# NoahVl/Explaining-In-Style-Reproducibility-Study

Hardware: AMD Instinct MI355X
Metric: StylEx G+D+enc train-step images/sec @256px (higher is better)
Workload: dtype bf16; 1 GPU; FFHQ-shaped 256x256 StylEx, batch 32/GPU, GAE=2 (noise+encoder micro-steps), GP every 4th step, ResNet-18 classifier; image_size=256, batch_per_gpu=32, start_step=0, gradient_accumulate_every=2, global_batch=32, parallelism=dp1

## Files before the change

explaining-in-style-reproducibility-study_amd/csrc/fused_bwd.hip:

```cpp
#include <hip/hip_runtime.h>
#include <stdint.h>
#include <stdlib.h>

#include "stylex_internal.h"

namespace {

constexpr int NT = 256;

template <int K>
struct Acc {
    float4 v[K];
    __device__ __forceinline__ void zero() {
#pragma unroll
        for (int k = 0; k < K; ++k) v[k] = make_float4(0.f, 0.f, 0.f, 0.f);
    }
};

template <int K>
__device__ __forceinline__ void block_reduce_store(Acc<K>& a, float* smem, int cv, int prow, int CV, int rpp, int C,
                                                   float* partial_row , bool active) {
    float4* s4 = reinterpret_cast<float4*>(smem);
    if (active) {
#pragma unroll
// ... 326 lines not shown
            const long o1 = two ? o + step : o;
            L8 t0 = ld8(t, o), t1 = ld8(t, o1);
            const L8 x0 = ld8(x, o), x1 = ld8(x, o1);
#pragma unroll
            for (int e = 0; e < 8; ++e) a[0].e[e] += x0.e[e] * t0.e[e];
            if (two) {
#pragma unroll
                for (int e = 0; e < 8; ++e) a[0].e[e] += x1.e[e] * t1.e[e];
            }
            if (gx) {
#pragma unroll
                for (int e = 0; e < 8; ++e) {
                    t0.e[e] *= s8.e[e];
                    t1.e[e] *= s8.e[e];
                }
                st8(gx, o, t0);
                if (two) st8(gx, o1, t1);
            }
        }
    }
    block_reduce_store8<1>(a, smem, g, C, partial + ((long)g.b * nchunks + blockIdx.x) * C);
}

inline size_t reduce_smem8(int C, int K) { return (size_t)K * (NT / (C >> 2)) * (C >> 3) * 32; }

inline bool al16(const void* p) { return (reinterpret_cast<uintptr_t>(p) & 15) == 0; }
inline bool glue_wide(int act_dtype, int C) {
    const char* env = getenv("STYLEX_GLUE_WIDE");
    return act_dtype == 1 && C % 8 == 0 && !(env && env[0] == '0');
}

inline size_t reduce_smem(int C, int K) {
    int CV = (C + 3) / 4;
    if (CV > NT) CV = NT;
    int rpp = NT / CV;
    return (size_t)K * rpp * CV * 16;
}

inline bool ok_shape(const int64_t* sh, int nchunks) {
    return sh[0] > 0 && sh[1] > 0 && sh[2] > 0 && sh[3] > 0 && sh[3] <= 1024 && (sh[3] % 4 == 0) && nchunks > 0 &&
           sh[0] <= 65535;
}

}

extern "C" {
// ... 60 lines not shown
        return (int)hipGetLastError();
    }
    hipLaunchKernelGGL(modconv_bwd_prep_kernel, dim3(nchunks, (unsigned)sh[0]), dim3(NT), reduce_smem(C, 3),
                       (hipStream_t)stream, gy, y, noise, (int)noise_stride, noise_w, noise_b, gz, partial, (int)sh[1],
                       (int)sh[2], C, nchunks, lrelu, act_dtype, gz_scale, natural);
    return (int)hipGetLastError();
}

int stylex_scale_reduce(const void* x, const void* t, const float* s, void* gx, float* partial, const int64_t* sh,
                        int nchunks, int act_dtype, void* stream) {
    if (act_dtype != 0 && act_dtype != 1) return STYLEX_EINVAL;
    if (!x || !t || !s || !partial || !ok_shape(sh, nchunks)) return STYLEX_EINVAL;
    int HW = (int)(sh[1] * sh[2]), C = (int)sh[3];
    if (glue_wide(act_dtype, C) && al16(x) && al16(t) && al16(s) && al16(gx) && al16(partial)) {
        hipLaunchKernelGGL(scale_reduce_wide_kernel, dim3(nchunks, (unsigned)sh[0]), dim3(NT8), reduce_smem8(C, 1),
                           (hipStream_t)stream, x, t, s, gx, partial, HW, C, nchunks);
        return (int)hipGetLastError();
    }
    hipLaunchKernelGGL(scale_reduce_kernel, dim3(nchunks, (unsigned)sh[0]), dim3(NT), reduce_smem(C, 1),
                       (hipStream_t)stream, x, t, s, gx, partial, HW, C, nchunks, act_dtype);
    return (int)hipGetLastError();
}

}
```

explaining-in-style-reproducibility-study_amd/stylex/hip_backend.py:

```python
import os as _os

if _os.environ.get("STYLEX_MIOPEN_ALLOW_BWD_GTC", "0") != "1":
    _os.environ.setdefault("MIOPEN_DEBUG_CONV_IMPLICIT_GEMM_ASM_BWD_GTC_XDLOPS_NHWC", "0")

import atexit
import ctypes
import os
import weakref

import torch

import operand_cache
from operand_cache import mark_updated, packs, stamp as _gen, vectors

_HERE = os.path.dirname(os.path.abspath(__file__))
LIB_PATH = os.path.join(os.path.dirname(_HERE), "libstylex_hip.so")

F32, BF16, BF16_ACT = 0, 1, 2
EPI_BIAS, EPI_LRELU, EPI_OSCALE, EPI_NOISE, EPI_RESIDUAL, EPI_RELU, EPI_GATE, EPI_NOISE_NAT = 1, 2, 4, 8, 16, 32, 64, 128
EPI_MASK_OUT, EPI_GATE_MASK = 256, 512

_c_f = ctypes.c_void_p
_i64p = ctypes.POINTER(ctypes.c_int64)

# ... 47 lines not shown
    "stylex_conv2d_bwd_weight_s2d": (ctypes.c_int, [ctypes.c_void_p, ctypes.c_void_p, _c_f, ctypes.c_void_p, ctypes.c_int64, _i64p,
                                                    ctypes.c_int, ctypes.c_float, ctypes.c_int, ctypes.c_int, ctypes.c_void_p]),
    "stylex_upsample2x_bilinear_fwd": (ctypes.c_int, [_c_f, _c_f, _i64p, ctypes.c_int, ctypes.c_void_p]),
    "stylex_upsample2x_bilinear_bwd": (ctypes.c_int, [_c_f, _c_f, _i64p, ctypes.c_int, ctypes.c_void_p]),
    "stylex_rgb_up_blur_add_fwd": (ctypes.c_int, [_c_f, _c_f, _c_f, _i64p, ctypes.c_int, ctypes.c_void_p]),
    "stylex_rgb_up_blur_add_bwd": (ctypes.c_int, [_c_f, _c_f, _i64p, ctypes.c_int, ctypes.c_void_p]),
    "stylex_blur3x3_reflect_fwd": (ctypes.c_int, [_c_f, _c_f, _i64p, ctypes.c_int, ctypes.c_void_p]),
    "stylex_blur3x3_reflect_bwd": (ctypes.c_int, [_c_f, _c_f, _i64p, ctypes.c_int, ctypes.c_void_p]),
    "stylex_bias_act_fwd": (ctypes.c_int, [_c_f, _c_f, _c_f, ctypes.c_int64, _c_f, _c_f, _c_f, _i64p, ctypes.c_int,
                                           ctypes.c_void_p]),
    "stylex_bias_act_bwd": (ctypes.c_int, [_c_f, _c_f, _c_f, _i64p, ctypes.c_int, ctypes.c_void_p]),
    "stylex_rowwise_sumsq": (ctypes.c_int, [_c_f, _c_f, _i64p, ctypes.c_void_p]),
    "stylex_reduce_chunks": (ctypes.c_int, [_i64p]),
    "stylex_act_bwd_reduce": (ctypes.c_int, [_c_f, _c_f, _c_f, _c_f, _i64p, ctypes.c_int, ctypes.c_int, ctypes.c_float,
                                             ctypes.c_int, ctypes.c_void_p]),
    "stylex_modconv_bwd_prep": (ctypes.c_int, [_c_f, _c_f, _c_f, ctypes.c_int64, _c_f, _c_f, _c_f, _c_f, _i64p,
                                               ctypes.c_int, ctypes.c_int, ctypes.c_int, ctypes.c_void_p]),
    "stylex_modconv_bwd_prep_scaled": (ctypes.c_int, [_c_f, _c_f, _c_f, ctypes.c_int64, _c_f, _c_f, _c_f, _c_f, _c_f, _i64p,
                                                      ctypes.c_int, ctypes.c_int, ctypes.c_int, ctypes.c_void_p]),
    "stylex_modconv_bwd_prep_nat": (ctypes.c_int, [_c_f, _c_f, _c_f, ctypes.c_int64, _c_f, _c_f, _c_f, _c_f, _c_f, _i64p,
                                                   ctypes.c_int, ctypes.c_int, ctypes.c_int, ctypes.c_void_p]),
    "stylex_scale_reduce": (ctypes.c_int, [_c_f, _c_f, _c_f, _c_f, _c_f, _i64p, ctypes.c_int, ctypes.c_int,
                                           ctypes.c_void_p]),
    "stylex_pad_rgb8": (ctypes.c_int, [_c_f, _c_f, _i64p, _i64p, ctypes.c_int, ctypes.c_void_p]),
    "stylex_affine_act_nchw_fwd": (ctypes.c_int, [_c_f, _c_f, _c_f, _c_f, _c_f, ctypes.c_int64, ctypes.c_int64, ctypes.c_int64,
                                                  ctypes.c_int, ctypes.c_void_p]),
    "stylex_affine_act_nchw_bwd": (ctypes.c_int, [_c_f, _c_f, _c_f, _c_f, _c_f, ctypes.c_int64, ctypes.c_int64, ctypes.c_int64,
                                                  ctypes.c_int, ctypes.c_void_p]),
    "stylex_affine_relu_maxpool_fwd": (ctypes.c_int, [_c_f, _c_f, _c_f, _c_f, _c_f, ctypes.c_int64, ctypes.c_int64,
                                                      ctypes.c_int64, ctypes.c_int64, ctypes.c_void_p]),
    "stylex_affine_relu_maxpool_bwd": (ctypes.c_int, [_c_f, _c_f, _c_f, _c_f, ctypes.c_int64, ctypes.c_int64, ctypes.c_int64,
                                                      ctypes.c_int64, ctypes.c_void_p]),
    "stylex_lpips_tap_nhwc_fwd": (ctypes.c_int, [_c_f, _c_f, _c_f, _c_f, _c_f, _c_f, ctypes.c_int64, ctypes.c_int64, ctypes.c_int64,
                                                 ctypes.c_int64, ctypes.c_void_p]),
    "stylex_lpips_tap_nhwc_bwd": (ctypes.c_int, [_c_f, _c_f, _c_f, _c_f, _c_f, _c_f, _c_f, _c_f, ctypes.c_int64, ctypes.c_int64,
                                                 ctypes.c_int64, ctypes.c_void_p]),
    "stylex_nchw_f32_to_nhwc_bf16": (ctypes.c_int, [_c_f, _c_f, ctypes.c_int64, ctypes.c_int64, ctypes.c_int64, ctypes.c_int,
                                                    ctypes.c_void_p]),
    "stylex_nhwc_bf16_to_nchw_f32": (ctypes.c_int, [_c_f, _c_f, _c_f, ctypes.c_int64, ctypes.c_int64, ctypes.c_int64, ctypes.c_void_p]),
    "stylex_resize_norm_fwd": (ctypes.c_int, [_c_f, _c_f, _c_f, _c_f, _i64p, _i64p, ctypes.c_void_p]),
    "stylex_resize_norm_bwd": (ctypes.c_int, [_c_f, _c_f, _c_f, _i64p, ctypes.c_void_p]),
    "stylex_fid_prep": (ctypes.c_int, [_c_f, _c_f, _i64p, _i64p, ctypes.c_int, ctypes.c_void_p]),
    "stylex_affine_act_nchw_slice_fwd": (ctypes.c_int, [_c_f, _c_f, _c_f, _c_f, _c_f, ctypes.c_int64, ctypes.c_int64,
                                                        ctypes.c_int64, ctypes.c_int64, ctypes.c_int, ctypes.c_void_p]),
    "stylex_fid_moments_acc": (ctypes.c_int, [_c_f, _c_f, _c_f, _c_f, ctypes.c_int64, ctypes.c_int64, ctypes.c_int64,
                                              ctypes.c_void_p]),
# ... 70 lines not shown
    "stylex_initial_block_bwd_data": (ctypes.c_int, [_c_f, _c_f, _c_f, _i64p, ctypes.c_int, ctypes.c_int, ctypes.c_void_p]),
    "stylex_initial_block_bwd_weight": (ctypes.c_int, [_c_f, _c_f, _c_f, _i64p, ctypes.c_int, ctypes.c_void_p]),
    "stylex_resample_rows_u8": (ctypes.c_int, [ctypes.c_void_p, _c_f, ctypes.c_int64, ctypes.c_int64, ctypes.c_int64, _c_f,
                                               ctypes.c_int64, _c_f, ctypes.c_int64, ctypes.c_void_p]),
    "stylex_resample_cols_u8": (ctypes.c_int, [ctypes.c_void_p, _c_f, ctypes.c_int64, ctypes.c_int64, ctypes.c_int64, _c_f,
                                               ctypes.c_int64, _c_f, ctypes.c_int64, _c_f, _c_f, ctypes.c_int64,
                                               ctypes.c_void_p]),
    "stylex_crop_lut_u8": (ctypes.c_int, [ctypes.c_void_p, _c_f, ctypes.c_int64, ctypes.c_int64, ctypes.c_int64, _c_f,
                                          ctypes.c_int64, _c_f, _c_f, ctypes.c_int64, ctypes.c_void_p]),
    "stylex_style_edit_max_k": (ctypes.c_int64, []),
    "stylex_style_edit_levels": (ctypes.c_int, [_c_f] * 9 + [ctypes.c_int64] * 5 + [ctypes.c_float, ctypes.c_void_p]),
    "stylex_timing_report": (ctypes.c_int, [ctypes.c_int, _i64p, ctypes.POINTER(ctypes.c_double),
                                            ctypes.POINTER(ctypes.c_double), ctypes.POINTER(ctypes.c_double)]),
}

_lib = None
_inited_devices = set()


class StylexHipError(RuntimeError):
    pass


OPTIONAL_SYMBOLS = frozenset(["stylex_modconv_bwd_prep_nat"])
_MISSING_OPTIONAL = set()


def has_symbol(name):
    load_library()
    return name not in _MISSING_OPTIONAL


def load_library(path=None):
    global _lib
    if _lib is not None:
        return _lib
    path = path or os.environ.get("STYLEX_HIP_LIB", LIB_PATH)
    if not os.path.isfile(path):
        raise StylexHipError("libstylex_hip.so not found at %s — run `python __graft_entry__.py build` "
                             "(there is no CPU fallback for the product path)" % path)
    lib = ctypes.CDLL(path)
    _MISSING_OPTIONAL.clear()
    for name, (res, args) in SIGNATURES.items():
        if name in OPTIONAL_SYMBOLS and path != LIB_PATH and not hasattr(lib, name):
            _MISSING_OPTIONAL.add(name)
            continue
        fn = getattr(lib, name)
# ... 1401 lines not shown
                                           _ptr(partial), shp, nch, lr, _adt(gy), _stream()), "stylex_modconv_bwd_prep")
    else:
        gz_scale = _f32(gz_scale)
        _check(lib.stylex_modconv_bwd_prep_scaled(_ptr(gy), _ptr(y), _ptr(noise), ns, _ptr(noise_w), _ptr(noise_b),
                                                  _ptr(gz_scale), _ptr(gz), _ptr(partial), shp, nch, lr, _adt(gy), _stream()),
               "stylex_modconv_bwd_prep_scaled")
    return gz, partial.sum(dim=1)


def scale_reduce(x, t, s, want_gx=True):
    lib = _ensure_device(x)
    assert is_cl(x) and is_cl(t) and x.dtype == t.dtype
    b, c, h, w = x.shape
    shp = _shape(b, h, w, c)
    nch = lib.stylex_reduce_chunks(shp)
    partial = _empty((b, nch, c), dtype=torch.float32, device=x.device)
    gx = empty_cl(tuple(x.shape), x) if want_gx else None
    s = _f32(s)
    _check(lib.stylex_scale_reduce(_ptr(x), _ptr(t), _ptr(s), _ptr(gx), _ptr(partial), shp, nch, _adt(x), _stream()),
           "stylex_scale_reduce")
    return gx, partial.sum(dim=1)


def torgb_ok(x):
    c = x.shape[1]
    if os.environ.get("STYLEX_TORGB", "1") == "0":
        return False
    return x.is_cuda and x.dtype == torch.bfloat16 and 8 <= c <= 512 and (c & (c - 1)) == 0


def torgb_fwd(x, s1, w):
    lib = _ensure_device(x)
    assert is_cl(x) and x.dtype == torch.bfloat16
    b, c, h, wd = x.shape
    y = empty_cl((b, 4, h, wd), x)
    s1, w = _f32(s1), _f32(w)
    _check(lib.stylex_torgb_fwd(_ptr(x), _ptr(s1), _ptr(w), _ptr(y), _shape(b, h, wd, c), _stream()), "stylex_torgb_fwd")
    return y


def torgb_bwd(x, gy, s1, w, want_gx=True):
    lib = _ensure_device(x)
    assert is_cl(x) and is_cl(gy) and gy.shape[1] == 4 and x.dtype == gy.dtype == torch.bfloat16
    b, c, h, wd = x.shape
    shp = _shape(b, h, wd, c)
    nch = lib.stylex_torgb_chunks(shp)
# ... 316 lines not shown
```

explaining-in-style-reproducibility-study_amd/stylex/networks.py:

```python
import atexit
import math
from math import log2

import os

import torch
import torch.nn.functional as F
from torch import nn

import ops


def exists(v):
    return v is not None


_SIDE = {}
atexit.register(_SIDE.clear)


def _side_stream(t, which=0):
    import os

    if not t.is_cuda or os.environ.get("STYLEX_STREAMS", "1") == "0":
# ... 222 lines not shown

    def forward_main(self, x, istyle, inoise, styles=None):
        if exists(self.upsample):
            x = self.upsample(x)
        coords = None
        self._rgb_style = None
        if styles is None:
            fused = ops.style_affines(istyle, self.to_style1, self.to_style2, self.to_rgb.to_style)
            if fused is not None:
                style1, style2, self._rgb_style, coords = fused
            else:
                style1, style2 = self.to_style1(istyle), self.to_style2(istyle)
        else:
            style1, style2 = styles
        x = ops.modconv_noise_act(x, style1, self.conv1.weight, inoise, self.to_noise1.weight[:, 0],
                                  self.to_noise1.bias, demod=self.conv1.demod, eps=self.conv1.eps)
        x = ops.modconv_noise_act(x, style2, self.conv2.weight, inoise, self.to_noise2.weight[:, 0],
                                  self.to_noise2.bias, demod=self.conv2.demod, eps=self.conv2.eps)
        return x, (coords if coords is not None else torch.cat([style1, style2], dim=-1))

    def forward(self, x, prev_rgb, istyle, inoise):
        x, coords = self.forward_main(x, istyle, inoise)
        rgb = self.to_rgb(x, prev_rgb, istyle, style=self.__dict__.pop("_rgb_style", None))
        return x, rgb, coords


class DiscriminatorBlock(nn.Module):
    def __init__(self, input_channels, filters, downsample=True):
        super().__init__()
        self.conv_res = HipConv2d(input_channels, filters, 1, stride=(2 if downsample else 1))
        self.net = nn.Sequential(HipConv2d(input_channels, filters, 3, padding=1, act=True), _FusedAct(),
                                 HipConv2d(filters, filters, 3, padding=1, act=True), _FusedAct())
        self.downsample = nn.Sequential(Blur(), HipConv2d(filters, filters, 3, padding=1, stride=2)) if downsample else None

    def forward(self, x):
        fused = getattr(ops.impl(), "dblock", None)
        if fused is not None:
            out = fused(x, self.conv_res, self.net[0], self.net[2], self.downsample[1] if exists(self.downsample) else None)
            if out is not None:
                return out
        side = _side_stream(x)
        if side is None:
            res = self.conv_res(x)
            x = self.net(x)
        else:
            main = torch.cuda.current_stream()
# ... 35 lines not shown
            self.initial_block = nn.Parameter(torch.randn((1, filters[0], 4, 4)))
        self.initial_conv = HipConv2d(filters[0], filters[0], 3, padding=1)
        self.blocks = nn.ModuleList([])
        self.attns = nn.ModuleList([])
        for ind in range(self.num_layers):
            self.attns.append(attn_and_ff(filters[ind]) if self.num_layers - ind in attn_layers else None)
            self.blocks.append(GeneratorBlock(latent_dim, filters[ind], filters[ind + 1], upsample=ind != 0,
                                              upsample_rgb=ind != self.num_layers - 1, rgba=transparent))

    def first_activation(self, styles):
        if self.no_const:
            return ops.initial_block(styles, self.to_initial_block.weight)
        return self.initial_block.expand(styles.shape[0], -1, -1, -1)

    def forward(self, styles, input_noise, get_style_coords=False, block_inputs=None):
        x = self.initial_conv(self.first_activation(styles))
        rgb, coords = None, []
        per_layer = styles.unbind(1)
        for li, block in enumerate(self.blocks):
            if exists(self.attns[li]):
                x = self.attns[li](x)
            if block_inputs is not None:
                block_inputs.append((x, rgb))
            x, sc = block.forward_main(x, per_layer[li], input_noise)
            coords.append(sc)
            rgb = block.to_rgb(x, rgb, per_layer[li], style=block.__dict__.pop("_rgb_style", None), padded=True)
        if rgb.shape[1] == 4 and self.blocks[0].to_rgb.conv.filters == 3:
            rgb = rgb[:, :3]
        rgb = rgb.float()
        if get_style_coords:
            return rgb, torch.cat(coords, dim=1)
        return rgb


class DiscriminatorE(nn.Module):
    def __init__(self, image_size, network_capacity=16, fq_layers=[], fq_dict_size=256, attn_layers=[],
                 transparent=False, encoder=False, encoder_dim=512, fmap_max=512, conditional=False):
        super().__init__()
        assert not fq_layers, "the fq variant is out of scope (SURVEY §2a)"
        filters = discriminator_filters(image_size, network_capacity, fmap_max, transparent)
        n = len(filters) - 1
        blocks, attn_blocks = [], []
        for i in range(n):
            blocks.append(DiscriminatorBlock(filters[i], filters[i + 1], downsample=i != n - 1))
            attn_blocks.append(attn_and_ff(filters[i + 1]) if i + 1 in attn_layers else None)
        self.blocks = nn.ModuleList(blocks)
        self.attn_blocks = nn.ModuleList(attn_blocks)
        self.quantize_blocks = nn.ModuleList([None] * n)
        chan_last = filters[-1]
# ... 20 lines not shown
```

explaining-in-style-reproducibility-study_amd/stylex/ops.py:

```python
import collections
import math

import os

import torch
from contextlib import nullcontext as _nullcontext
import torch.nn.functional as F

import hip_backend as hb

_PRECISION = hb.F32


_NAMES = {"fp32": hb.F32, "f32": hb.F32, "bf16": hb.BF16_ACT, "bf16_f32act": hb.BF16}


def set_precision(name):
    global _PRECISION
    _PRECISION = _NAMES[name]


def get_precision():
    return {hb.F32: "fp32", hb.BF16_ACT: "bf16", hb.BF16: "bf16_f32act"}[_PRECISION]

# ... 478 lines not shown


def _natural_noise(inoise):
    hit = _NAT_NOISE.get("k")
    if (hit is not None and hit[0] is inoise and hit[1] == inoise._version
            and not (inoise.is_cuda and torch.cuda.is_current_stream_capturing())):
        return hit[2]
    nat = inoise[:, :, :, 0].transpose(1, 2).contiguous().float()
    _NAT_NOISE["k"] = (inoise, inoise._version, nat)
    return nat


class _ModConvFast(torch.autograd.Function):

    @staticmethod
    def forward(ctx, x, s1, d, w, noise, nw, nb, pad, lrelu, noise_nat=None):
        x = _cl(x)
        pre = _PRECISION == hb.BF16_ACT and s1 is not None and x.shape[2] * x.shape[3] <= 64 and x.shape[1] % 64 == 0
        ctx.pre = pre
        if pre:
            x_in, s_in = (x.float() * s1[:, :, None, None]).to(x.dtype).contiguous(memory_format=torch.channels_last), None
        else:
            x_in, s_in = x, s1
        if noise_nat is not None and noise_nat.shape[1] % 4 == 0:
            y = hb.conv2d_fwd(x_in, w, 1, pad, _PRECISION, in_scale=s_in, out_scale=d, noise=noise_nat, noise_w=nw,
                              noise_b=nb, lrelu=lrelu, noise_natural=True)
        else:
            y = hb.conv2d_fwd(x_in, w, 1, pad, _PRECISION, in_scale=s_in, out_scale=d, noise=noise, noise_w=nw, noise_b=nb,
                              lrelu=lrelu)
        ctx.save_for_backward(x, s1, d, w, noise, nw, nb, y if (lrelu or d is not None or noise is not None) else None,
                              noise_nat)
        ctx.cfg = (pad, lrelu)
        return y

    @staticmethod
    @torch.autograd.function.once_differentiable
    def backward(ctx, gy):
        x, s1, d, w, noise, nw, nb, y, noise_nat = ctx.saved_tensors
        pad, lrelu = ctx.cfg
        gy = _cl(gy)
        gd = gnw = gnb = None
        folded = False
        if y is not None and _reducible(gy.shape[1]):
            fold = d is not None and _PRECISION != hb.F32 and os.environ.get("STYLEX_FOLD_D", "1") != "0"
            if noise_nat is not None and hb.has_symbol("stylex_modconv_bwd_prep_nat"):
                gz, sums = hb.modconv_bwd_prep(gy, y, noise_nat, nw, nb, lrelu, gz_scale=d if fold else None,
                                               noise_natural=True)
            else:
                gz, sums = hb.modconv_bwd_prep(gy, y, noise, nw, nb, lrelu, gz_scale=d if fold else None)
            folded = fold
            if d is not None:
                gd = sums[:, 0] / d
# ... 279 lines not shown
        else:
            gx += gxs
        if cin == 3:
            gx = gx[:, :3]
    return (gx, gw_res, gsum3, gw1, gb1, gw2, gb2, gw3, gsum3 if plan.downsample else None), (gz3, gz2, gz1)


class _DBlockFast(torch.autograd.Function):

    @staticmethod
    def forward(ctx, x, w_res, b_res, w1, b1, w2, b2, w3, b3, downsample):
        out, ctx.plan, saved = _dblock_forward(x, (w_res, b_res, w1, b1, w2, b2, w3, b3), downsample)
        ctx.save_for_backward(*saved)
        return out

    @staticmethod
    @torch.autograd.function.once_differentiable
    def backward(ctx, g_out):
        need = ctx.needs_input_grad
        grads, _ = _dblock_backward(ctx.plan, _DBlockSaved(*ctx.saved_tensors), g_out, need)
        return tuple(g if wanted else None for g, wanted in zip(grads, need)) + (None,)


_GACC = {}
_GACC_TASK = [-2]
_GACC_ON = os.environ.get("STYLEX_GRAD_ACC", "1") != "0"
_GACC_STREAMS = set()
_GACC_WAITED = {}
_GACC_SEQ = [0]


def _gacc_join():
    if _GACC_STREAMS:
        cur = torch.cuda.current_stream()
        for st in _GACC_STREAMS:
            if st != cur:
                cur.wait_stream(st)
        _GACC_STREAMS.clear()


def _gacc_get(w, tag=""):
    if not _GACC_ON or not w.is_cuda:
        return None
    task = torch._C._current_graph_task_id()
    if task < 0:
        return None
# ... 130 lines not shown
                and w % 2 == 0 and w // 2 >= 16 and h // 2 >= 16 and tuple(weight.shape[2:]) == (3, 3)):
            x2 = _BlurS2D.apply(_act(x))
            if fast_enabled():
                return _DownS2DFast.apply(x2, weight, bias, _act(residual), res_scale)
            return _ConvBiasActDD.apply(x2, weight, bias, _act(residual), 1, 1, False, res_scale, c)
        return HipOps.conv2d(HipOps.blur3x3(x), weight, bias, stride=2, padding=1, residual=residual,
                             res_scale=res_scale)

    @staticmethod
    def rgb_block(x, prev_rgb, style, weight, upsample):
        if not fast_enabled() or os.environ.get("STYLEX_RGB_TAIL", "1") == "0":
            return None
        x = _act(x)
        if tuple(weight.shape[2:]) != (1, 1) or weight.shape[0] != 3 or not hb.torgb_ok(x):
            return None
        if prev_rgb is not None and (prev_rgb.shape[1] != 4 or prev_rgb.dtype != x.dtype):
            return None
        rgb = _ToRGBFast.apply(x, style + 1, weight)
        if upsample:
            return _RGBTailFast.apply(rgb, prev_rgb)
        return rgb if prev_rgb is None else rgb + prev_rgb

    @staticmethod
    def residual_merge(x, res):
        return (x + res) * (1 / math.sqrt(2))

    @staticmethod
    def dblock(x, conv_res, conv1, conv2, down):
        if not fast_enabled() or os.environ.get("STYLEX_DBLOCK", "1") == "0":
            return None
        if conv1.weight.shape[0] % 4 != 0:
            return None
        return _DBlockFast.apply(x, conv_res.weight, conv_res.bias, conv1.weight, conv1.bias, conv2.weight, conv2.bias,
                                 down.weight if down is not None else None, down.bias if down is not None else None,
                                 down is not None)

    @staticmethod
    def style_edit_levels(coords, smin, smax, sindex, direction, base_class, level_k, seg_start, shift_size):
        return hb.style_edit_levels(coords, smin, smax, sindex, direction, base_class, level_k, seg_start, shift_size)

    @staticmethod
    def rowwise_sumsq(x2d):
        return _RowSumSq.apply(x2d)


_IMPL = HipOps
# ... 131 lines not shown


def modconv_noise_act(*a, **k):
    return _IMPL.modconv_noise_act(*a, **k)


def upsample2x(x):
    return _IMPL.upsample2x(x)


def blur3x3(x):
    return _IMPL.blur3x3(x)


def blur_down(*a, **k):
    return _IMPL.blur_down(*a, **k)


def rgb_block(*a, **k):
    fn = getattr(_IMPL, "rgb_block", None)
    return fn(*a, **k) if fn is not None else None


def residual_merge(x, res):
    return _IMPL.residual_merge(x, res)


def rowwise_sumsq(x2d):
    return _IMPL.rowwise_sumsq(x2d)



_ATTN_FUSED = os.environ.get("STYLEX_ATTN_FUSED", "1") != "0"


def set_attn_fused(flag):
    global _ATTN_FUSED
    prev = _ATTN_FUSED
    _ATTN_FUSED = bool(flag)
    return prev


def _wide(t):
    return t.float() if t.dtype in (torch.bfloat16, torch.float16) else t


# ... 202 lines not shown
```

include/stylex_hip.h:

```cpp
#ifndef STYLEX_HIP_H
#define STYLEX_HIP_H

#include <stdint.h>

#ifdef __cplusplus
extern "C" {
#endif

#define STYLEX_F32 0
#define STYLEX_BF16 1
#define STYLEX_BF16_ACT 2

#define STYLEX_EINVAL (-1)
#define STYLEX_EWORKSPACE (-2)

#define STYLEX_CONV_NSHAPE 11

#define STYLEX_EPI_BIAS 1
#define STYLEX_EPI_LRELU 2
#define STYLEX_EPI_OSCALE 4
#define STYLEX_EPI_NOISE 8
#define STYLEX_EPI_RESIDUAL 16
#define STYLEX_EPI_RELU 32
#define STYLEX_EPI_NOISE_NAT 128
// ... 147 lines not shown
int stylex_weight_sumsq(const float* w, float* wsq, int64_t O, int64_t C, int64_t K, void* stream);
int stylex_modcoeff_fwd(const float* style, const float* wsq, float* s1, float* d, int64_t B, int64_t C, int64_t O,
                        float eps, void* stream);
int stylex_modcoeff_bwd(const float* gd, const float* d, const float* s1, const float* wsq, const float* w,
                        const float* gs1, float* gstyle, float* gw, int64_t B, int64_t C, int64_t O, int64_t K,
                        void* stream);

int stylex_reduce_chunks(const int64_t* shape);
int stylex_act_bwd_reduce(const void* dy, const void* y, void* dx, float* partial, const int64_t* shape, int nchunks,
                          int lrelu, float scale, int act_dtype, void* stream);
int stylex_modconv_bwd_prep(const void* gy, const void* y, const float* noise, int64_t noise_stride,
                            const float* noise_w, const float* noise_b, void* gz, float* partial,
                            const int64_t* shape, int nchunks, int lrelu, int act_dtype, void* stream);
int stylex_modconv_bwd_prep_scaled(const void* gy, const void* y, const float* noise, int64_t noise_stride,
                                   const float* noise_w, const float* noise_b, const float* gz_scale, void* gz,
                                   float* partial, const int64_t* shape, int nchunks, int lrelu, int act_dtype,
                                   void* stream);
int stylex_modconv_bwd_prep_nat(const void* gy, const void* y, const float* noise, int64_t noise_stride,
                                const float* noise_w, const float* noise_b, const float* gz_scale, void* gz,
                                float* partial, const int64_t* shape, int nchunks, int lrelu, int act_dtype,
                                void* stream);
int stylex_scale_reduce(const void* x, const void* t, const float* s, void* gx, float* partial, const int64_t* shape,
                        int nchunks, int act_dtype, void* stream);

int stylex_torgb_chunks(const int64_t* shape);
int stylex_torgb_fwd(const void* x, const float* s1, const float* w, void* y, const int64_t* shape, void* stream);
int stylex_torgb_bwd(const void* x, const void* gy, const float* s1, const float* w, void* gx, float* partial,
                     const int64_t* shape, void* stream);

int stylex_timing_enable(int on);
int stylex_timing_pause(int on);
int stylex_timing_report(int kernel_class, int64_t* launches, double* total_ms, double* total_flops,
                         double* total_bytes);
int stylex_timing_layers(int64_t* meta, double* vals, int64_t cap);
int stylex_timing_kernels(char* names, int64_t* meta, double* vals, int64_t cap);

#define STYLEX_ADAM_COPY_PACK 0
#define STYLEX_ADAM_COPY_PACK_S2D 1
#define STYLEX_ADAM_COPY_SUMSQ 2
typedef struct {
    float* p;
    const float* g;
    float* m;
    float* v;
    const float* step;
    int64_t numel;
// ... 77 lines not shown
```

Measured before the change: 1016 images/sec.

## Fuse generator block backward seams into single-pass prep kernels via custom autograd

Adds a whole-generator-block autograd function (two modulated convs plus toRGB) whose backward fuses two elementwise seams into new wide bf16 kernels. The toRGB gradient is combined with the incoming gradient inside the modconv backward prep. The scale-reduce of the second conv's data gradient is merged with the first conv's prep. This removes intermediate gradient tensors and separate elementwise passes over activations, at the cost of extra rounding steps to mirror the old bf16 materialisation. Blocks adjacent to attention layers fall back to the old path.

```diff
diff --git a/explaining-in-style-reproducibility-study_amd/csrc/fused_bwd.hip b/explaining-in-style-reproducibility-study_amd/csrc/fused_bwd.hip
--- a/explaining-in-style-reproducibility-study_amd/csrc/fused_bwd.hip
+++ b/explaining-in-style-reproducibility-study_amd/csrc/fused_bwd.hip
@@ -372,6 +372,154 @@
     block_reduce_store8<1>(a, smem, g, C, partial + ((long)g.b * nchunks + blockIdx.x) * C);
 }
 
+__device__ __forceinline__ L8 round8(const L8& v) {
+    L8 r;
+#pragma unroll
+    for (int i = 0; i < 4; ++i) {
+        const unsigned u = act_pack2(v.e[2 * i], v.e[2 * i + 1]);
+        r.e[2 * i] = act_lo(u);
+        r.e[2 * i + 1] = act_hi(u);
+    }
+    return r;
+}
+struct RgbM {
+    float m[3][8];
+};
+__device__ __forceinline__ L8 rgb_gx(const uint2 g, const RgbM& k) {
+    const float g0 = act_lo(g.x), g1 = act_hi(g.x), g2 = act_lo(g.y);
+    L8 v;
+#pragma unroll
+    for (int e = 0; e < 8; ++e) v.e[e] = __fmaf_rn(g2, k.m[2][e], __fmaf_rn(g0, k.m[0][e], __fmul_rn(g1, k.m[1][e])));
+    return round8(v);
+}
+
+enum { SEAM_SUM = 0, SEAM_SCALE = 1 };
+struct SeamSrc {
+    const void* g;
+    const uint2* g_rgb;
+    const float* s3;
+    const float* w3;
+    const float* s;
+    float* partial_sr;
+};
+
+template <int SEAM>
+__global__ __launch_bounds__(NT8) void gblock_prep_wide_kernel(SeamSrc src, const void* __restrict__ y,
+                                                             const float* __restrict__ noise, int ns,
+                                                             const float* __restrict__ nw, const float* __restrict__ nb,
+                                                             void* __restrict__ gz, float* __restrict__ partial, int H, int W,
+                                                             int C, int nchunks, int lrelu, const float* __restrict__ gz_scale,
+                                                             int natural) {
+    extern __shared__ __attribute__((aligned(16))) float smem[];
+    const int HW = H * W;
+    const Geo8 g = make_geo8(HW, C, nchunks);
+    L8 a[3] = {};
+    L8 asr[1] = {};
+    if (g.active) {
+        const int c = g.cv * 8;
+        L8 w8 = {}, b8 = {}, d8 = {}, s8 = {};
+        RgbM k = {};
+        if (noise) {
+            w8 = ldp8(nw + c);
+            b8 = ldp8(nb + c);
+        }
+        if (gz_scale) d8 = ldp8(gz_scale + (long)g.b * C + c);
+        if (SEAM == SEAM_SCALE) {
+            s8 = ldp8(src.s + (long)g.b * C + c);
+        } else {
+#pragma unroll
+            for (int e = 0; e < 8; ++e) {
+                const float sv = src.s3[(long)g.b * C + c + e];
+#pragma unroll
+                for (int n = 0; n < 3; ++n) k.m[n][e] = __fmul_rn(src.w3[n * C + c + e], sv);
+            }
+        }
+        const long step = (long)g.rpp * C;
+        const long pix0 = (long)g.b * HW;
+        long o = (pix0 + g.p_begin + g.prow) * C + c;
+        PixWalk pw(g.p_begin + g.prow, g.rpp, W);
+        for (int p = g.p_begin + g.prow; p < g.p_end; p += 2 * g.rpp, o += 2 * step, pw.advance()) {
+            const bool two = p + g.rpp < g.p_end;
+            const long o1 = two ? o + step : o;
+            const int p1 = two ? p + g.rpp : p;
+            const int h0 = pw.h, w0 = pw.w;
+            pw.advance();
+            const int h1 = two ? pw.h : h0, w1 = two ? pw.w : w0;
+            const L8 y0 = ld8(y, o), y1 = ld8(y, o1);
+            L8 g0, g1;
+            if (SEAM == SEAM_SCALE) {
+                const L8 t0 = ld8(src.g, o), t1 = ld8(src.g, o1);
+#pragma unroll
+                for (int e = 0; e < 8; ++e) asr[0].e[e] += y0.e[e] * t0.e[e];
+                if (two) {
+#pragma unroll
+                    for (int e = 0; e < 8; ++e) asr[0].e[e] += y1.e[e] * t1.e[e];
+                }
+#pragma unroll
+                for (int e = 0; e < 8; ++e) {
+                    g0.e[e] = __fmul_rn(t0.e[e], s8.e[e]);
+                    g1.e[e] = __fmul_rn(t1.e[e], s8.e[e]);
+                }
+                g0 = round8(g0);
+                g1 = round8(g1);
+            } else {
+                g0 = rgb_gx(src.g_rgb[pix0 + p], k);
+                g1 = rgb_gx(src.g_rgb[pix0 + p1], k);
+                if (src.g) {
+                    const L8 n0 = ld8(src.g, o), n1 = ld8(src.g, o1);
+#pragma unroll
+                    for (int e = 0; e < 8; ++e) {
+                        g0.e[e] = __fadd_rn(g0.e[e], n0.e[e]);
+                        g1.e[e] = __fadd_rn(g1.e[e], n1.e[e]);
+                    }
+                    g0 = round8(g0);
+                    g1 = round8(g1);
+                }
+            }
+            float nz0 = 0.f, nz1 = 0.f;
+            if (noise) {
+                nz0 = noise[noise_off(g.b, ns, h0, w0, natural)];
+                nz1 = noise[noise_off(g.b, ns, h1, w1, natural)];
+            }
+            L8 q0, q1, t0 = y0, t1 = y1, s0, s1;
+#pragma unroll
+            for (int e = 0; e < 8; ++e) {
+                q0.e[e] = g0.e[e];
+                q1.e[e] = g1.e[e];
+                if (lrelu) {
+                    q0.e[e] = y0.e[e] > 0.f ? g0.e[e] : 0.2f * g0.e[e];
+                    t0.e[e] = y0.e[e] > 0.f ? y0.e[e] : 5.f * y0.e[e];
+                    q1.e[e] = y1.e[e] > 0.f ? g1.e[e] : 0.2f * g1.e[e];
+                    t1.e[e] = y1.e[e] > 0.f ? y1.e[e] : 5.f * y1.e[e];
+                }
+                s0.e[e] = gz_scale ? q0.e[e] * d8.e[e] : q0.e[e];
+                s1.e[e] = gz_scale ? q1.e[e] * d8.e[e] : q1.e[e];
+            }
+            st8(gz, o, s0);
+            if (two) st8(gz, o1, s1);
+#pragma unroll
+            for (int e = 0; e < 8; ++e) {
+                a[0].e[e] += q0.e[e] * (t0.e[e] - (nz0 * w8.e[e] + b8.e[e]));
+                a[1].e[e] += q0.e[e] * nz0;
+                a[2].e[e] += q0.e[e];
+            }
+            if (two) {
+#pragma unroll
+                for (int e = 0; e < 8; ++e) {
+                    a[0].e[e] += q1.e[e] * (t1.e[e] - (nz1 * w8.e[e] + b8.e[e]));
+                    a[1].e[e] += q1.e[e] * nz1;
+                    a[2].e[e] += q1.e[e];
+                }
+            }
+        }
+    }
+    if (SEAM == SEAM_SCALE) {
+        block_reduce_store8<1>(asr, smem, g, C, src.partial_sr + ((long)g.b * nchunks + blockIdx.x) * C);
+        __syncthreads();
+    }
+    block_reduce_store8<3>(a, smem, g, C, partial + ((long)g.b * nchunks + blockIdx.x) * 3 * C);
+}
+
 inline size_t reduce_smem8(int C, int K) { return (size_t)K * (NT / (C >> 2)) * (C >> 3) * 32; }
 
 inline bool al16(const void* p) { return (reinterpret_cast<uintptr_t>(p) & 15) == 0; }
@@ -478,4 +626,53 @@
     return (int)hipGetLastError();
 }
 
-}
+static int seam_prep_args(const void* y, const float* noise, int64_t noise_stride, const float* noise_w,
+                          const float* noise_b, const float* gz_scale, int natural, const void* gz, const float* partial,
+                          const int64_t* sh, int nchunks, int lrelu, int act_dtype) {
+    if (act_dtype != 0 && act_dtype != 1) return STYLEX_EINVAL;
+    if (lrelu != 0 && lrelu != 1) return STYLEX_EINVAL;
+    if (natural != 0 && natural != 1) return STYLEX_EINVAL;
+    if (!y || !gz || !partial || !ok_shape(sh, nchunks)) return STYLEX_EINVAL;
+    if (noise && (!noise_w || !noise_b || noise_stride < sh[1] || noise_stride < sh[2])) return STYLEX_EINVAL;
+    if (natural && !noise) return STYLEX_EINVAL;
+    if (!glue_wide(act_dtype, (int)sh[3]) || !al16(y) || !al16(gz) || !al16(partial) || !al16(noise_w) || !al16(noise_b) ||
+        !al16(gz_scale))
+        return STYLEX_NOT_APPLICABLE;
+    return 0;
+}
+
+int stylex_modconv_bwd_prep_sum(const void* g_next, const void* g_rgb, const float* s3, const float* w3, const void* y,
+                                const float* noise, int64_t noise_stride, const float* noise_w, const float* noise_b,
+                                const float* gz_scale, int natural, void* gz, float* partial, const int64_t* sh, int nchunks,
+                                int lrelu, int act_dtype, void* stream) {
+    if (!g_rgb || !s3 || !w3) return STYLEX_EINVAL;
+    const int rc = seam_prep_args(y, noise, noise_stride, noise_w, noise_b, gz_scale, natural, gz, partial, sh, nchunks,
+                                  lrelu, act_dtype);
+    if (rc) return rc;
+    if (!al16(g_next) || (reinterpret_cast<uintptr_t>(g_rgb) & 7)) return STYLEX_NOT_APPLICABLE;
+    const int C = (int)sh[3];
+    SeamSrc src = {g_next, (const uint2*)g_rgb, s3, w3, nullptr, nullptr};
+    hipLaunchKernelGGL(gblock_prep_wide_kernel<SEAM_SUM>, dim3(nchunks, (unsigned)sh[0]), dim3(NT8), reduce_smem8(C, 3),
+                       (hipStream_t)stream, src, y, noise, (int)noise_stride, noise_w, noise_b, gz, partial, (int)sh[1],
+                       (int)sh[2], C, nchunks, lrelu, gz_scale, natural);
+    return (int)hipGetLastError();
+}
+
+int stylex_scale_reduce_prep(const void* y, const void* t, const float* s, const float* noise, int64_t noise_stride,
+                             const float* noise_w, const float* noise_b, const float* gz_scale, int natural, void* gz,
+                             float* partial_sr, float* partial, const int64_t* sh, int nchunks, int lrelu, int act_dtype,
+                             void* stream) {
+    if (!t || !s || !partial_sr) return STYLEX_EINVAL;
+    const int rc = seam_prep_args(y, noise, noise_stride, noise_w, noise_b, gz_scale, natural, gz, partial, sh, nchunks,
+                                  lrelu, act_dtype);
+    if (rc) return rc;
+    if (!al16(t) || !al16(s) || !al16(partial_sr)) return STYLEX_NOT_APPLICABLE;
+    const int C = (int)sh[3];
+    SeamSrc src = {t, nullptr, nullptr, nullptr, s, partial_sr};
+    hipLaunchKernelGGL(gblock_prep_wide_kernel<SEAM_SCALE>, dim3(nchunks, (unsigned)sh[0]), dim3(NT8), reduce_smem8(C, 3),
+                       (hipStream_t)stream, src, y, noise, (int)noise_stride, noise_w, noise_b, gz, partial, (int)sh[1],
+                       (int)sh[2], C, nchunks, lrelu, gz_scale, natural);
+    return (int)hipGetLastError();
+}
+
+}
diff --git a/explaining-in-style-reproducibility-study_amd/stylex/hip_backend.py b/explaining-in-style-reproducibility-study_amd/stylex/hip_backend.py
--- a/explaining-in-style-reproducibility-study_amd/stylex/hip_backend.py
+++ b/explaining-in-style-reproducibility-study_amd/stylex/hip_backend.py
@@ -93,6 +93,10 @@
                                                    ctypes.c_int, ctypes.c_int, ctypes.c_int, ctypes.c_void_p]),
     "stylex_scale_reduce": (ctypes.c_int, [_c_f, _c_f, _c_f, _c_f, _c_f, _i64p, ctypes.c_int, ctypes.c_int,
                                            ctypes.c_void_p]),
+    "stylex_modconv_bwd_prep_sum": (ctypes.c_int, [_c_f] * 6 + [ctypes.c_int64, _c_f, _c_f, _c_f, ctypes.c_int, _c_f, _c_f, _i64p,
+                                                   ctypes.c_int, ctypes.c_int, ctypes.c_int, ctypes.c_void_p]),
+    "stylex_scale_reduce_prep": (ctypes.c_int, [_c_f] * 4 + [ctypes.c_int64, _c_f, _c_f, _c_f, ctypes.c_int, _c_f, _c_f, _c_f, _i64p,
+                                                ctypes.c_int, ctypes.c_int, ctypes.c_int, ctypes.c_void_p]),
     "stylex_pad_rgb8": (ctypes.c_int, [_c_f, _c_f, _i64p, _i64p, ctypes.c_int, ctypes.c_void_p]),
     "stylex_affine_act_nchw_fwd": (ctypes.c_int, [_c_f, _c_f, _c_f, _c_f, _c_f, ctypes.c_int64, ctypes.c_int64, ctypes.c_int64,
                                                   ctypes.c_int, ctypes.c_void_p]),
@@ -209,7 +213,7 @@
     pass
 
 
-OPTIONAL_SYMBOLS = frozenset(["stylex_modconv_bwd_prep_nat"])
+OPTIONAL_SYMBOLS = frozenset(["stylex_modconv_bwd_prep_nat", "stylex_modconv_bwd_prep_sum", "stylex_scale_reduce_prep"])
 _MISSING_OPTIONAL = set()
 
 
@@ -1657,6 +1661,49 @@
     return gx, partial.sum(dim=1)
 
 
+NOT_APPLICABLE = -100
+
+
+def _seam_prep_args(y, noise, noise_w, noise_b, gz_scale):
+    b, c, h, w = y.shape
+    shp = _shape(b, h, w, c)
+    nch = load_library().stylex_reduce_chunks(shp)
+    partial = _empty((b, nch, 3, c), dtype=torch.float32, device=y.device)
+    gz = empty_cl(tuple(y.shape), y)
+    noise, noise_w, noise_b, gz_scale = _f32(noise), _f32(noise_w), _f32(noise_b), _f32(gz_scale)
+    return shp, nch, partial, gz, noise, noise_w, noise_b, gz_scale, (noise.shape[1] if noise is not None else 0)
+
+
+def modconv_bwd_prep_sum(g_next, g_rgb, s3, w3, y, noise, noise_w, noise_b, lrelu, gz_scale=None, noise_natural=False):
+    lib = _ensure_device(y)
+    assert is_cl(y) and is_cl(g_rgb) and g_rgb.shape[1] == 4 and g_rgb.dtype == y.dtype
+    assert g_next is None or (is_cl(g_next) and g_next.dtype == y.dtype and g_next.shape == y.shape)
+    shp, nch, partial, gz, noise, noise_w, noise_b, gz_scale, ns = _seam_prep_args(y, noise, noise_w, noise_b, gz_scale)
+    s3, w3 = _f32(s3), _f32(w3)
+    rc = lib.stylex_modconv_bwd_prep_sum(_ptr(g_next), _ptr(g_rgb), _ptr(s3), _ptr(w3), _ptr(y), _ptr(noise), ns, _ptr(noise_w),
+                                         _ptr(noise_b), _ptr(gz_scale), int(bool(noise_natural)), _ptr(gz), _ptr(partial), shp,
+                                         nch, int(bool(lrelu)), _adt(y), _stream())
+    if rc == NOT_APPLICABLE:
+        return None
+    _check(rc, "stylex_modconv_bwd_prep_sum")
+    return gz, partial.sum(dim=1)
+
+
+def scale_reduce_prep(y, t, s, noise, noise_w, noise_b, lrelu, gz_scale=None, noise_natural=False):
+    lib = _ensure_device(y)
+    assert is_cl(y) and is_cl(t) and t.dtype == y.dtype and t.shape == y.shape
+    shp, nch, partial, gz, noise, noise_w, noise_b, gz_scale, ns = _seam_prep_args(y, noise, noise_w, noise_b, gz_scale)
+    partial_sr = _empty((y.shape[0], nch, y.shape[1]), dtype=torch.float32, device=y.device)
+    s = _f32(s)
+    rc = lib.stylex_scale_reduce_prep(_ptr(y), _ptr(t), _ptr(s), _ptr(noise), ns, _ptr(noise_w), _ptr(noise_b), _ptr(gz_scale),
+                                      int(bool(noise_natural)), _ptr(gz), _ptr(partial_sr), _ptr(partial), shp, nch,
+                                      int(bool(lrelu)), _adt(y), _stream())
+    if rc == NOT_APPLICABLE:
+        return None
+    _check(rc, "stylex_scale_reduce_prep")
+    return gz, partial.sum(dim=1), partial_sr.sum(dim=1)
+
+
 def torgb_ok(x):
     c = x.shape[1]
     if os.environ.get("STYLEX_TORGB", "1") == "0":
diff --git a/explaining-in-style-reproducibility-study_amd/stylex/networks.py b/explaining-in-style-reproducibility-study_amd/stylex/networks.py
--- a/explaining-in-style-reproducibility-study_amd/stylex/networks.py
+++ b/explaining-in-style-reproducibility-study_amd/stylex/networks.py
@@ -268,6 +268,27 @@
     def forward(self, x, prev_rgb, istyle, inoise):
         x, coords = self.forward_main(x, istyle, inoise)
         rgb = self.to_rgb(x, prev_rgb, istyle, style=self.__dict__.pop("_rgb_style", None))
+        return x, rgb, coords
+
+    def forward_padded(self, x, prev_rgb, istyle, inoise, fuse=True):
+        rgb_conv = self.to_rgb.conv
+        h, w = (2 * x.shape[2], 2 * x.shape[3]) if exists(self.upsample) else tuple(x.shape[2:])
+        plan = ops.gblock_plan((x.shape[0], x.shape[1], h, w), x.is_cuda, self.conv1, self.conv2, rgb_conv,
+                               prev_rgb) if fuse else None
+        if plan is None:
+            x, coords = self.forward_main(x, istyle, inoise)
+            return x, self.to_rgb(x, prev_rgb, istyle, style=self.__dict__.pop("_rgb_style", None), padded=True), coords
+        if exists(self.upsample):
+            x = self.upsample(x)
+        fused = ops.style_affines(istyle, self.to_style1, self.to_style2, self.to_rgb.to_style)
+        if fused is not None:
+            style1, style2, rgb_style, coords = fused
+        else:
+            style1, style2, rgb_style = self.to_style1(istyle), self.to_style2(istyle), self.to_rgb.to_style(istyle)
+            coords = torch.cat([style1, style2], dim=-1)
+        x, rgb = ops.gblock(plan, x, prev_rgb, style1, style2, rgb_style, self.conv1, self.conv2, rgb_conv, inoise,
+                            (self.to_noise1.weight[:, 0], self.to_noise1.bias), (self.to_noise2.weight[:, 0], self.to_noise2.bias),
+                            exists(self.to_rgb.upsample))
         return x, rgb, coords
 
 
@@ -349,9 +370,9 @@
                 x = self.attns[li](x)
             if block_inputs is not None:
                 block_inputs.append((x, rgb))
-            x, sc = block.forward_main(x, per_layer[li], input_noise)
+            lone = not exists(self.attns[li]) and not (li + 1 < self.num_layers and exists(self.attns[li + 1]))
+            x, rgb, sc = block.forward_padded(x, rgb, per_layer[li], input_noise, fuse=lone)
             coords.append(sc)
-            rgb = block.to_rgb(x, rgb, per_layer[li], style=block.__dict__.pop("_rgb_style", None), padded=True)
         if rgb.shape[1] == 4 and self.blocks[0].to_rgb.conv.filters == 3:
             rgb = rgb[:, :3]
         rgb = rgb.float()
diff --git a/explaining-in-style-reproducibility-study_amd/stylex/ops.py b/explaining-in-style-reproducibility-study_amd/stylex/ops.py
--- a/explaining-in-style-reproducibility-study_amd/stylex/ops.py
+++ b/explaining-in-style-reproducibility-study_amd/stylex/ops.py
@@ -524,12 +524,7 @@
             x_in, s_in = (x.float() * s1[:, :, None, None]).to(x.dtype).contiguous(memory_format=torch.channels_last), None
         else:
             x_in, s_in = x, s1
-        if noise_nat is not None and noise_nat.shape[1] % 4 == 0:
-            y = hb.conv2d_fwd(x_in, w, 1, pad, _PRECISION, in_scale=s_in, out_scale=d, noise=noise_nat, noise_w=nw,
-                              noise_b=nb, lrelu=lrelu, noise_natural=True)
-        else:
-            y = hb.conv2d_fwd(x_in, w, 1, pad, _PRECISION, in_scale=s_in, out_scale=d, noise=noise, noise_w=nw, noise_b=nb,
-                              lrelu=lrelu)
+        y = _modconv_noise_fwd(x_in, s_in, d, w, noise, nw, nb, pad, lrelu, noise_nat, _PRECISION)
         ctx.save_for_backward(x, s1, d, w, noise, nw, nb, y if (lrelu or d is not None or noise is not None) else None,
                               noise_nat)
         ctx.cfg = (pad, lrelu)
@@ -855,6 +850,114 @@
         return tuple(g if wanted else None for g, wanted in zip(grads, need)) + (None,)
 
 
+
+_GBlockPlan = collections.namedtuple("_GBlockPlan", "prec pad fold nat_bwd")
+_GBlockSaved = collections.namedtuple(
+    "_GBlockSaved", "u y1 y2 s1a da w1 nw1 nb1 s1b db w2 nw2 nb2 s3 w3 noise noise_nat")
+
+
+def _gblock_plan(u_shape, u_dtype, u_cuda, w_shapes, prec, has_seams=None):
+    if os.environ.get("STYLEX_GBLOCK_FUSE", "1") == "0" or prec != hb.BF16_ACT or not u_cuda or u_dtype != torch.bfloat16:
+        return None
+    (n1, c1, k1, _), (n2, c2, k2, _), w3 = w_shapes
+    b, cin, h, w = u_shape
+    if cin != c1 or n1 != c2 or n2 != n1 or k1 != k2 or k1 % 2 != 1 or tuple(w3) != (3, n2, 1, 1):
+        return None
+    if n1 % 8 != 0 or not _reducible(cin) or h * w <= 64:
+        return None
+    if not (8 <= n2 <= 512 and (n2 & (n2 - 1)) == 0) or os.environ.get("STYLEX_TORGB", "1") == "0":
+        return None
+    if has_seams is None:
+        has_seams = hb.has_symbol("stylex_modconv_bwd_prep_sum") and hb.has_symbol("stylex_scale_reduce_prep")
+    if not has_seams:
+        return None
+    return _GBlockPlan(prec, (k1 - 1) // 2, os.environ.get("STYLEX_FOLD_D", "1") != "0", hb.has_symbol("stylex_modconv_bwd_prep_nat"))
+
+
+def _modconv_noise_fwd(x, s1, d, w, noise, nw, nb, pad, lrelu, noise_nat, prec):
+    if noise_nat is not None and noise_nat.shape[1] % 4 == 0:
+        return hb.conv2d_fwd(x, w, 1, pad, prec, in_scale=s1, out_scale=d, noise=noise_nat, noise_w=nw, noise_b=nb,
+                             lrelu=lrelu, noise_natural=True)
+    return hb.conv2d_fwd(x, w, 1, pad, prec, in_scale=s1, out_scale=d, noise=noise, noise_w=nw, noise_b=nb, lrelu=lrelu)
+
+
+def _gblock_forward(plan, u, s1a, da, w1, nw1, nb1, s1b, db, w2, nw2, nb2, s3, w3, noise, noise_nat):
+    u = _cl(u)
+    y1 = _modconv_noise_fwd(u, s1a, da, w1, noise, nw1, nb1, plan.pad, True, noise_nat, plan.prec)
+    y2 = _modconv_noise_fwd(y1, s1b, db, w2, noise, nw2, nb2, plan.pad, True, noise_nat, plan.prec)
+    rgb = hb.torgb_fwd(y2, s3, w3)
+    return (y2, rgb), _GBlockSaved(u, y1, y2, s1a, da, w1, nw1, nb1, s1b, db, w2, nw2, nb2, s3, w3, noise, noise_nat)
+
+
+def _gblock_backward(plan, sv, g_next, g_rgb, need):
+    prec, pad, fold = plan.prec, plan.pad, plan.fold
+    nat = sv.noise_nat is not None and plan.nat_bwd
+    plane = sv.noise_nat if nat else sv.noise
+    g_next = _cl(g_next) if g_next is not None else None
+
+    def prep(gy, y, nw, nb, d):
+        return hb.modconv_bwd_prep(gy, y, plane, nw, nb, True, gz_scale=d if fold else None, noise_natural=nat)
+
+    def conv_grads(x, gz, w, s1, d, want_t, want_w):
+        t = gw = None
+        if want_t:
+            t = hb.conv2d_bwd_data(gz, w, tuple(x.shape), 1, pad, prec, in_scale=None if fold else d)
+        if want_w:
+            gw = hb.conv2d_bwd_weight(x, gz, tuple(w.shape), 1, pad, prec, x_scale=s1, dy_scale=None if fold else d)
+        return t, gw
+
+    gs3 = gw3 = seam = None
+    if g_rgb is not None:
+        g_rgb = _cl(g_rgb)
+        seam = hb.modconv_bwd_prep_sum(g_next, g_rgb, sv.s3, sv.w3, sv.y2, plane, sv.nw2, sv.nb2, True,
+                                       gz_scale=sv.db if fold else None, noise_natural=nat)
+        gx_rgb, t3 = hb.torgb_bwd(sv.y2, g_rgb, sv.s3, sv.w3, want_gx=seam is None)
+        if need[11]:
+            gs3 = (t3 * sv.w3.reshape(1, 3, -1).float()).sum(dim=1)
+        if need[12]:
+            gw3 = (t3 * sv.s3.float()[:, None, :]).sum(dim=0).reshape(sv.w3.shape).to(sv.w3.dtype)
+        if seam is None:
+            g_next = gx_rgb if g_next is None else gx_rgb + g_next
+    gz2, sums2 = seam if seam is not None else prep(g_next, sv.y2, sv.nw2, sv.nb2, sv.db)
+    gdb = sums2[:, 0] / sv.db
+    gnw2, gnb2 = sums2[:, 1:3].sum(0)
+    t2, gw2 = conv_grads(sv.y1, gz2, sv.w2, sv.s1b, sv.db, True, need[8])
+    seam = hb.scale_reduce_prep(sv.y1, t2, sv.s1b, plane, sv.nw1, sv.nb1, True, gz_scale=sv.da if fold else None,
+                                noise_natural=nat)
+    if seam is None:
+        gx1, gs1b = hb.scale_reduce(sv.y1, t2, sv.s1b, want_gx=True)
+        gz1, sums1 = prep(gx1, sv.y1, sv.nw1, sv.nb1, sv.da)
+    else:
+        gz1, sums1, gs1b = seam
+    gda = sums1[:, 0] / sv.da
+    gnw1, gnb1 = sums1[:, 1:3].sum(0)
+    t1, gw1 = conv_grads(sv.u, gz1, sv.w1, sv.s1a, sv.da, need[0] or need[1], need[3])
+    gu = gs1a = None
+    if t1 is not None:
+        gu, gs1a = hb.scale_reduce(sv.u, t1, sv.s1a, want_gx=need[0])
+    return gu, gs1a, gda, gw1, gnw1, gnb1, gs1b, gdb, gw2, gnw2, gnb2, gs3, gw3
+
+
+class _GBlockFast(torch.autograd.Function):
+
+    @staticmethod
+    def forward(ctx, plan, u, s1a, da, w1, nw1, nb1, s1b, db, w2, nw2, nb2, s3, w3, noise, noise_nat):
+        out, saved = _gblock_forward(plan, u, s1a, da, w1, nw1, nb1, s1b, db, w2, nw2, nb2, s3, w3, noise, noise_nat)
+        ctx.plan = plan
+        ctx.set_materialize_grads(False)
+        ctx.save_for_backward(*saved)
+        return out
+
+    @staticmethod
+    @torch.autograd.function.once_differentiable
+    def backward(ctx, g_next, g_rgb):
+        need = ctx.needs_input_grad[1:14]
+        if g_next is None and g_rgb is None:
+            return (None,) * 16
+        grads = _gblock_backward(ctx.plan, _GBlockSaved(*ctx.saved_tensors), g_next, g_rgb, need)
+        return (None,) + tuple(g if wanted else None for g, wanted in zip(grads, need)) + (None, None)
+
+
 _GACC = {}
 _GACC_TASK = [-2]
 _GACC_ON = os.environ.get("STYLEX_GRAD_ACC", "1") != "0"
@@ -1031,6 +1134,29 @@
         return rgb if prev_rgb is None else rgb + prev_rgb
 
     @staticmethod
+    def gblock_plan(u_shape, u_cuda, conv1, conv2, rgb_conv, prev_rgb):
+        if not fast_enabled() or os.environ.get("STYLEX_RGB_TAIL", "1") == "0":
+            return None
+        if not (conv1.demod and conv2.demod) or rgb_conv.demod:
+            return None
+        adt = hb.act_dtype(_PRECISION)
+        if prev_rgb is not None and (prev_rgb.shape[1] != 4 or prev_rgb.dtype != adt):
+            return None
+        return _gblock_plan(tuple(u_shape), adt, u_cuda, [tuple(c.weight.shape) for c in (conv1, conv2, rgb_conv)], _PRECISION)
+
+    @staticmethod
+    def gblock(plan, u, prev_rgb, style1, style2, rgb_style, conv1, conv2, rgb_conv, inoise, noise1, noise2, upsample_rgb):
+        u = _act(u)
+        s1a, da = mod_coeffs(style1, conv1.weight, True, conv1.eps)
+        s1b, db = mod_coeffs(style2, conv2.weight, True, conv2.eps)
+        nat = _natural_noise(inoise) if os.environ.get("STYLEX_NOISE_NAT", "1") != "0" else None
+        y2, rgb = _GBlockFast.apply(plan, u, s1a, da, conv1.weight, noise1[0], noise1[1], s1b, db, conv2.weight, noise2[0],
+                                    noise2[1], rgb_style + 1, rgb_conv.weight, inoise[:, :, :, 0], nat)
+        if upsample_rgb:
+            return y2, _RGBTailFast.apply(rgb, prev_rgb)
+        return y2, (rgb if prev_rgb is None else rgb + prev_rgb)
+
+    @staticmethod
     def residual_merge(x, res):
         return (x + res) * (1 / math.sqrt(2))
 
@@ -1208,6 +1334,15 @@
     return fn(*a, **k) if fn is not None else None
 
 
+def gblock_plan(*a, **k):
+    fn = getattr(_IMPL, "gblock_plan", None)
+    return fn(*a, **k) if fn is not None else None
+
+
+def gblock(*a, **k):
+    return _IMPL.gblock(*a, **k)
+
+
 def residual_merge(x, res):
     return _IMPL.residual_merge(x, res)
 
diff --git a/include/stylex_hip.h b/include/stylex_hip.h
--- a/include/stylex_hip.h
+++ b/include/stylex_hip.h
@@ -193,6 +193,14 @@
                                 void* stream);
 int stylex_scale_reduce(const void* x, const void* t, const float* s, void* gx, float* partial, const int64_t* shape,
                         int nchunks, int act_dtype, void* stream);
+int stylex_modconv_bwd_prep_sum(const void* g_next, const void* g_rgb, const float* s3, const float* w3, const void* y,
+                                const float* noise, int64_t noise_stride, const float* noise_w, const float* noise_b,
+                                const float* gz_scale, int natural, void* gz, float* partial, const int64_t* shape,
+                                int nchunks, int lrelu, int act_dtype, void* stream);
+int stylex_scale_reduce_prep(const void* y, const void* t, const float* s, const float* noise, int64_t noise_stride,
+                             const float* noise_w, const float* noise_b, const float* gz_scale, int natural, void* gz,
+                             float* partial_sr, float* partial, const int64_t* shape, int nchunks, int lrelu, int act_dtype,
+                             void* stream);
 
 int stylex_torgb_chunks(const int64_t* shape);
 int stylex_torgb_fwd(const void* x, const float* s1, const float* w, void* y, const int64_t* shape, void* stream);
```

Measured after the change: 1018 images/sec, median of 2. About the same (+0.2%).
